# omroot/DeepLearningInAssetPricing_PaperReplication

Measured on AMD Instinct MI355X. Metric: epochs/sec (3-phase GAN), higher is better.
Workload: dtype bf16; 1 GPU; model=Chen-Pelger-Zhu GAN: LSTM[4] + SDF FFN[64,64] + 8 tanh moments, global_batch=1, seq_len=240, panel=T=240/60/300 N=3000 F=46 M=178, bench_config=real, wide_layer0=False, models_per_gpu=1, parallelism=ensemble-dp1, backend=none

## Files before the change

csrc/engine.cpp:

```cpp
#include <cstdint>
#include <cstdlib>
#include <hip/hip_runtime.h>
#include <pybind11/numpy.h>
#include <pybind11/pybind11.h>
#include <pybind11/stl.h>

#include <execinfo.h>
#include <signal.h>
#include <sys/syscall.h>
#include <unistd.h>

#include <atomic>
#include <cmath>
#include <cstring>
#include <map>
#include <memory>
#include <mutex>
#include <stdexcept>
#include <string>
#include <vector>

#include <chrono>

#include "engine_plan.h"
// ... 1472 lines not shown
      launch_mlp_bwd_mom(as<MlpJob>(dh ? j_mlp_bwd_dh_ : j_mlp_bwd_[phase]), G_, gx_bwd_, md_.nslice_m, 1, md_.md,
                         md_.KS1, md_.WMB, slab_stride(), fpw_, st_);
    else
      launch_sdf_bwd(as<MlpJob>(j_mlp_bwd_[phase]));
    if (md_.md.wide)
      launch_wgrad0(as<WideJob>(j_wide_bwd_[phase]), G_, dd(), md_.md, phase == 2, md_.WMB, nsplit_, st_);
    enqueue_train_tail(tp);
  }
  long split_rows(int s) const { return splits_[s].R; }

  void set_stream(uintptr_t st, bool external) {
    HTRACE("set_stream %p ext=%d tid=%ld", (void*)st, (int)external, (long)syscall(SYS_gettid));
    hipStream_t want = external ? reinterpret_cast<hipStream_t>(st) : own_st_;
    if (want == st_ && external == ext_stream_) return;
    sync();
    st_ = want;
    ext_stream_ = external;
  }
  void join_from(uintptr_t ext) {
    HIP_OK(hipEventRecord(ev_[EV_IN], reinterpret_cast<hipStream_t>(ext)));
    HIP_OK(hipStreamWaitEvent(st_, ev_[EV_IN], 0));
  }
  void join_to(uintptr_t ext) {
    HIP_OK(hipEventRecord(ev_[EV_OUT], st_));
    HIP_OK(hipStreamWaitEvent(reinterpret_cast<hipStream_t>(ext), ev_[EV_OUT], 0));
  }
  void set_params_dev(int g, uintptr_t src) {
    check_g(g);
    HIP_OK(hipMemcpyAsync(models_[g].params.p, reinterpret_cast<const void*>(src), md_.P * sizeof(float),
                          hipMemcpyDeviceToDevice, st_));
    pack(g, false);
    h_valid_ = false;
  }
  void set_drop_step(int g, int step) { launch_set_int(models_[check_g(g)].drop_step.p, step, st_); }
  long copy_ws(int g, int s, const std::string& name, uintptr_t dst) {
    ModelSplitWS& W = ws(g, s);
    const std::map<std::string, DevBuf<float>*> m = {
        {"wn", &W.wn}, {"h", &W.h}, {"P", &W.P}, {"port", &W.port}, {"scal", &W.scal}, {"pp", &W.pp},
        {"w", &W.w}};
    auto it = m.find(name);
    if (it == m.end()) throw std::invalid_argument("copy_ws: unknown buffer " + name);
    const DevBuf<float>& b = *it->second;
    if (b.n) HIP_OK(hipMemcpyAsync(reinterpret_cast<void*>(dst), b.p, b.n * sizeof(float), hipMemcpyDeviceToDevice, st_));
    return (long)b.n;
  }
  void copy_grads(int g, uintptr_t dst) {
    HIP_OK(hipMemcpyAsync(reinterpret_cast<void*>(dst), models_[check_g(g)].grads.p, md_.P * sizeof(float),
                          hipMemcpyDeviceToDevice, st_));
  }
  void set_hidden(int g, int s, uintptr_t h, uintptr_t c) {
    ModelSplitWS& W = ws(check_g(g), s);
    const size_t n = (size_t)md_.nrnn * md_.H;
    if (n == 0) return;
    if (h) HIP_OK(hipMemcpyAsync(W.h0.p, reinterpret_cast<const void*>(h), n * 4, hipMemcpyDeviceToDevice, st_));
    else HIP_OK(hipMemsetAsync(W.h0.p, 0, n * 4, st_));
    if (c) HIP_OK(hipMemcpyAsync(W.c0.p, reinterpret_cast<const void*>(c), n * 4, hipMemcpyDeviceToDevice, st_));
    else HIP_OK(hipMemsetAsync(W.c0.p, 0, n * 4, st_));
  }
  void copy_hidden_grad(int g, uintptr_t dh, uintptr_t dc) {
    ModelSplitWS& W = ws(check_g(g), 0);
    const size_t n = (size_t)md_.nrnn * md_.H;
    if (n == 0) return;
    HIP_OK(hipMemcpyAsync(reinterpret_cast<void*>(dh), W.dh0.p, n * 4, hipMemcpyDeviceToDevice, st_));
    HIP_OK(hipMemcpyAsync(reinterpret_cast<void*>(dc), W.dc0.p, n * 4, hipMemcpyDeviceToDevice, st_));
  }
  void copy_hidden(int g, uintptr_t dst_h, uintptr_t dst_c) {
// ... 186 lines not shown
    int gx = std::max(gx_fwd_[1], gx_fwd_[2]);
    if (k_.eval_gx > 0) gx = std::min(gx, k_.eval_gx);
    return gx;
  }
  int train_fwd_grid(int phase) const { return phase == 2 ? gx_fwd_[0] : gx_fwd13_; }
  int ne_per_model() const { return G_ > 0 && n_eval_jobs_ % G_ == 0 ? n_eval_jobs_ / G_ : 0; }
  int tmax_fwd_all() const { return std::max(splits_[0].T, tmax_eval_); }
  bool fused_eval(const EvalPass& ep) const {
    return (k_.rnn_overlap_eval || ep.solo || ep.sep) && plan_[1].eval_fusable;
  }
  void plan_phases() {
    const bool overlap = k_.rnn_overlap && !safe_mode_ && md_.nrnn > 0 && !md_.md.wide;
    auto fits = [&](int T) { return mlp_fwd_rnn_supported(md_.md, md_.KS1, md_.WMB, md_.H, md_.nrnn, T); };
    const bool have0 = splits_[0].set, packs = inv_code_.p != nullptr;
    const int eval_gx = fused_grid(eval_grid(), n_eval_jobs_, cap_eval_), ne = ne_per_model();
    const bool eval_fusable = overlap && n_eval_jobs_ > 0 && fits(tmax_eval_) && eval_gx > 0;
    for (int phase = 1; phase <= 3; ++phase) {
      PhasePlan p;
      p.eval_gx_solo = eval_gx;
      p.eval_fusable = eval_fusable;
      const int gx = fused_grid(train_fwd_grid(phase), G_, cap_train_);
      p.fused_fwd = (phase != 2 || k_.fused_p2) && overlap && fits(splits_[0].T) && gx > 0;
      p.train_gx = p.fused_fwd ? gx : 0;
      p.selfproj = p.fused_fwd && k_.self_proj && !train_mom(phase);
      const int gxa = cap_all_ > 0 && ne > 0 ? std::min(train_fwd_grid(phase), cap_all_ / G_ - 1 - ne) : 0;
      p.eval_in_fwd = k_.eval_in_fwd && phase != 2 && ne > 0 && p.fused_fwd && fits(tmax_fwd_all()) && gxa >= 16;
      p.all_gx = p.eval_in_fwd ? gxa : 0;
      p.sep_eval = k_.eval_sep && phase != 2 && p.fused_fwd && eval_fusable;
      p.tail_fused = k_.fused_tail && !xs_on_ && phase != 2 && have0 && lstm_tail_supported(md_, splits_[0].T);
      const int nadam = (md_.P_sdf + ADAM_PB - 1) / ADAM_PB;
      p.adam_in_tail = k_.tail_adam != 0 && !safe_mode_ && p.tail_fused && packs && tail_cap_ > 0 &&
                       2 * G_ * nadam <= tail_cap_;
      p.split_graphs = k_.split_graphs && !safe_mode_ && p.adam_in_tail && (p.sep_eval || p.eval_in_fwd);
      p.mom_tail = phase == 2 && k_.mom_tail && !xs_on_ && packs && have0 && mom_tail_supported(md_, splits_[0].T) &&
                   !mlstm();
      p.p2_lstm_cached = phase == 2 && k_.p2_lstm_cache && md_.nrnn > 0 && (md_.nrnn == 1 || md_.dropout == 0.f) &&
                         !xs_on_;
      plan_[phase] = p;
    }
  }
  RunMode run_mode(int phase) const {
    const PhasePlan& p = plan_[phase];
    RunMode m;
    m.pipe = phase != 2 && n_eval_jobs_ > 0 && pipeline_;
    m.split = m.pipe && p.split_graphs;
    m.sep = m.split && p.sep_eval;
    m.tail_adam = m.split || (m.pipe && p.eval_in_fwd && k_.tail_adam == 2 && p.adam_in_tail);
    return m;
  }
 public:
  double capture_seconds() const { return capture_s_; }
  bool fused_fwd(int phase) const { return phase >= 1 && phase <= 3 && plan_[phase].fused_fwd; }
  void reset_prog_errors() {
    sync();
    std::vector<int> h((size_t)G_ * 3 * 16);
    HIP_LEGACY(hipMemcpy(h.data(), prog_.p, h.size() * sizeof(int), hipMemcpyDeviceToHost));
    for (int k = 0; k < 3 * G_; ++k) h[16 * k + 1] = 0;
    HIP_LEGACY(hipMemcpy(prog_.p, h.data(), h.size() * sizeof(int), hipMemcpyHostToDevice));
    for (ModelState& S : models_) {
      HIP_LEGACY(hipMemset(S.tail_ctr.p, 0, S.tail_ctr.n * sizeof(int)));
      HIP_LEGACY(hipMemset(S.upd_ctr.p, 0, S.upd_ctr.n * sizeof(int)));
    }
    HIP_LEGACY(hipMemset(esync_.p, 0, esync_.n * sizeof(int)));
  }
  py::dict fused_info() const {
    py::dict d;
    const RunMode m = run_mode(1);
    d["cap_train"] = cap_train_; d["cap_eval"] = cap_eval_;
    for (int ph = 1; ph <= 3; ++ph) d[("train_gx_p" + std::to_string(ph)).c_str()] = plan_[ph].train_gx;
    d["eval_gx_solo"] = plan_[1].eval_gx_solo;
    d["cap_all"] = cap_all_;
    d["tail_cap"] = tail_cap_;
    for (int ph = 1; ph <= 3; ph += 2) {
      d[("eval_in_fwd_p" + std::to_string(ph)).c_str()] = plan_[ph].eval_in_fwd;
      d[("all_gx_p" + std::to_string(ph)).c_str()] = plan_[ph].all_gx;
    }
    d["eval_per_model"] = ne_per_model();
    d["fused_tail"] = plan_[1].tail_fused;
    d["mom_tail"] = plan_[2].mom_tail;
    d["p2_lstm_cached"] = plan_[2].p2_lstm_cached;
    d["adam_in_tail"] = m.tail_adam && plan_[1].eval_in_fwd;
    d["split_graphs"] = m.split;
    d["eval_sep"] = m.sep;
    d["host_launch_us_per_epoch"] = host_launch_n_ ? 1e6 * host_launch_s_ / host_launch_n_ : 0.0;
    d["bwd_nfine"] = nfine_; d["bwd_fpw"] = fpw_;
    d["fused_pack"] = inv_code_.p != nullptr;
    d["bwd_lds_fpw1"] = (long)mlp_bwd_lds_bytes(md_.md, slab_stride(), 1);
    d["bwd_lds_fpw4"] = (long)mlp_bwd_lds_bytes(md_.md, slab_stride(), 4);
    return d;
  }
  int prog_timeouts() {
    sync();
    std::vector<int> h((size_t)G_ * 3 * 16);
    HIP_LEGACY(hipMemcpy(h.data(), prog_.p, h.size() * sizeof(int), hipMemcpyDeviceToHost));
    int n = 0;
    for (int k = 0; k < 3 * G_; ++k) n += h[16 * k + 1];
    return n;
  }
 private:
  bool train_mom(int phase) const { return phase == 2 || (phase == 3 && !cache_train_h()); }
  ModelDesc md_{};
  DevBuf<char> d_desc_;
  SplitDev splits_[3];
  std::vector<ModelState> models_;
  std::vector<ModelSplitWS> ws_;
  DevBuf<float> slab_;
  DevBuf<int> cnt_scratch_;
  DevBuf<float> nbar_scratch_;
  int nfine_ = 4;
  int fpw_ = 1;
  int slabs_stored() const { return nfine_ / fpw_; }
  int gx_bwd_ = 1, gx_fwd_[3] = {1, 1, 1};
  int gx_fwd13_ = 1;
  int nsplit_ = 1, gx_proj_[3] = {1, 1, 1};
  bool graphs_dirty_ = true;
  std::map<std::string, hipGraphExec_t> graphs_;
// ... 803 lines not shown
      HIP_OK(hipEventRecord(ev_[EV_MID], st_));
    } else {
      HTRACE("launch_job_metrics");
      launch_job_metrics(lj, G_, st_);
    }
    if (phase == 2) {
      HTRACE("launch_mlp_bwd_mom");
      launch_mlp_bwd_mom(as<MlpJob>(j_mlp_bwd_[phase]), G_, gx_bwd_, md_.nslice_m, 1, md_.md, md_.KS1,
                         md_.WMB, slab_stride(), fpw_, st_);
    } else {
      if (!tp.gram) {
        HTRACE("launch_period_bwd");
        launch_period_bwd(lj, G_, D.T, st_);
      }
      HTRACE("launch_mlp_bwd_sdf");
      launch_sdf_bwd(as<MlpJob>(j_mlp_bwd_[phase]));
    }
    if (md_.md.wide)
      launch_wgrad0(as<WideJob>(j_wide_bwd_[phase]), G_, dd(), md_.md, phase == 2, md_.WMB, nsplit_, st_);
    enqueue_train_tail(tp);
  }
  void enqueue_train_tail(const TrainPass& tp) {
    const int phase = tp.phase;
    const SplitDev& D = splits_[0];
    if (tp.mom_adam) {
      HTRACE("launch_lstm_tail(phase 2)");
      launch_lstm_tail(as<UpdJob>(j_upd_), as<FinJob>(j_fin_), G_, dd(), md_, D.T, slab_stride(), st_,
                       loss_tab(2, false), 1, tp.lr, 2);
      return;
    }
    const LossJob* lm = tp.tail_metrics && phase != 2 ? loss_tab(phase, tp.gram) : nullptr;
    if (plan_[phase].tail_fused) {
      HTRACE("launch_lstm_tail");
      launch_lstm_tail(as<UpdJob>(j_upd_), as<FinJob>(j_fin_), G_, dd(), md_, D.T, slab_stride(), st_, lm,
                       tp.tail_adam, tp.lr);
      return;
    }
    if (lm) launch_job_metrics(lm, G_, st_);
    HTRACE("launch_finalize");
    launch_finalize(as<FinJob>(j_fin_), G_, dd(), md_, phase, slab_stride(), D.T, st_);
    xs_call("grads", phase, st_);
    if (phase == 2 && mlstm()) {
      HTRACE("launch_mlstm_bwd");
      launch_mlstm_bwd(as<MlstmJob>(j_ml_train_), G_, D.T, dd(), md_, st_);
      return;
    }
    HTRACE("launch_lstm_bwd");
    launch_lstm_bwd(as<UpdJob>(j_upd_), G_, dd(), md_, D.T, phase, st_);
  }
  void enqueue_update(int phase, float lr) {
    HTRACE("launch_update");
    launch_update(as<UpdJob>(j_upd_), G_, dd(), md_, phase, lr, st_, inv_code_.p != nullptr);
  }
  void enqueue_train(int phase, float lr) {
    enqueue_train_grads(TrainPass(phase));
    enqueue_update(phase, lr);
  }
  void enqueue_eval(hipStream_t st, const EvalPass& ep) {
    enqueue_eval_prologue(st, ep);
    enqueue_eval_towers(st, ep);
  }
  void enqueue_eval_prologue(hipStream_t st, const EvalPass& ep) {
    if (n_eval_jobs_ == 0) return;
    HTRACE("launch_prologue");
    if (fused_eval(ep)) launch_proj(as<RnnJob>(j_rnn_eval_), n_eval_jobs_, tmax_eval_, dd(), md_, st, proj_abias(!k_.h_cache));
    else launch_prologue(as<RnnJob>(j_rnn_eval_), n_eval_jobs_, tmax_eval_, dd(), md_, st, proj_abias(!k_.h_cache));
    mom_table(j_ml_eval_, 0, n_eval_jobs_, tmax_eval_, st, !k_.h_cache, false);
  }
// ... 29 lines not shown
  void enqueue_eval_solo(int phase) {
    EvalPass ep = eval_pass(phase);
    ep.solo = true;
    enqueue_eval(st_, ep);
  }
  void enqueue_epoch_end(int phase, int ignore_epoch, float sel, hipStream_t st, int signal = 0) {
    HTRACE("launch_epoch_end");
    launch_epoch_end(as<EpochJob>(j_epoch_[phase]), G_, phase, ignore_epoch, sel, md_.residual_factor,
                     md_.P, st, signal);
  }
  void enqueue_epoch(int phase, float lr, int ignore_epoch, float sel, bool lstm_once) {
    TrainPass tp = epoch_pass(phase, lr);
    tp.mom_adam = plan_[phase].mom_tail;
    tp.lstm_once = lstm_once;
    enqueue_train_grads(tp);
    if (!tp.mom_adam) enqueue_update(phase, lr);
    if (phase != 2) enqueue_eval_solo(phase);
    enqueue_epoch_end(phase, ignore_epoch, sel, st_);
  }
  void enqueue_head(int phase, float lr, int part) {
    TrainPass tp = epoch_pass(phase, lr);
    tp.part = part;
    enqueue_train_grads(tp);
    enqueue_dropmask(phase, 1, st_);
    enqueue_update(phase, lr);
    if (plan_[phase].split_graphs && plan_[phase].sep_eval) launch_gen_sync(as<UpdJob>(j_upd_), G_, st_);
  }
  void enqueue_chain_split(int phase, float lr) {
    const bool sep = plan_[phase].sep_eval;
    TrainPass tp = epoch_pass(phase, lr);
    tp.premasked = true;
    tp.tail_metrics = true;
    tp.tail_adam = sep ? 3 : 2;
    tp.eval_rnn = !sep;
    tp.esig = sep ? nullptr : esync_.p;
    enqueue_train_grads(tp);
  }
  void enqueue_eval_split(int phase, int ignore_epoch, float sel) {
    EvalPass ep = eval_pass(phase);
    if (plan_[phase].sep_eval) {
      HTRACE("launch_wait_gen");
      launch_wait_gen(as<UpdJob>(j_upd_), G_, k_.spin_limit, st2_);
      ep.sep = true;
      ep.selfproj = k_.self_proj && k_.h_cache;
      if (!ep.selfproj) launch_proj(as<RnnJob>(j_rnn_eval_), n_eval_jobs_, tmax_eval_, dd(), md_, st2_, proj_abias(!k_.h_cache));
      mom_table(j_ml_eval_, 0, n_eval_jobs_, tmax_eval_, st2_, !k_.h_cache, false);
    } else {
      HTRACE("launch_wait_count");
      launch_wait_count(esync_.p, ne_per_model() * G_, k_.spin_limit, prog_.p, G_, st2_);
    }
    enqueue_eval_towers(st2_, ep);
    enqueue_dropmask(phase, 1, st2_);
    enqueue_epoch_end(phase, ignore_epoch, sel, st2_, 1);
  }
  void enqueue_pipe(int phase, float lr, int ignore_epoch, float sel) {
    HIP_OK(hipEventRecord(ev_[EV_FORK], st_));
    HIP_OK(hipStreamWaitEvent(st2_, ev_[EV_FORK], 0));
    TrainPass tp = epoch_pass(phase, lr);
    tp.premasked = true;
    const EvalPass ep = eval_pass(phase);
    if (plan_[phase].eval_in_fwd) {
      const bool ta = run_mode(phase).tail_adam;
      tp.eval_rnn = tp.mark_fwd = tp.tail_metrics = true;
      tp.tail_adam = ta ? 2 : 0;
      enqueue_train_grads(tp);
      HIP_OK(hipStreamWaitEvent(st2_, ev_[EV_FWD], 0));
      enqueue_eval_towers(st2_, ep);
      if (ta) {
        enqueue_dropmask(phase, 1, st2_);
        enqueue_epoch_end(phase, ignore_epoch, sel, st2_, 1);
        HIP_OK(hipEventRecord(ev_[EV_JOIN], st2_));
        HIP_OK(hipStreamWaitEvent(st_, ev_[EV_JOIN], 0));
        return;
      }
      enqueue_epoch_end(phase, ignore_epoch, sel, st2_);
      enqueue_dropmask(phase, 1, st2_);
    } else {
      tp.eval_prologue = st2_;
      tp.defer_metrics = true;
      enqueue_train_grads(tp);
      enqueue_eval_towers(st2_, ep);
      if (phase != 2) {
        HIP_OK(hipStreamWaitEvent(st2_, ev_[EV_MID], 0));
        launch_job_metrics(loss_tab(phase, tp.gram), G_, st2_);
      }
// ... 295 lines not shown
      .def("characteristic_gram", &Engine::characteristic_gram, py::arg("s"))
      .def("xgram_run", &Engine::xgram_run)
      .def("pred_loss", &Engine::pred_loss, py::arg("s"), py::arg("factor") = py::none(),
           py::arg("weighting") = "period", py::arg("refresh") = true, py::arg("write_dw") = false)
      .def("fit_begin", &Engine::fit_begin, py::arg("factors"), py::arg("weighting") = "period")
      .def("fit_epochs", &Engine::fit_epochs, py::arg("n"), py::arg("lr"), py::call_guard<py::gil_scoped_release>())
      .def("fit_history", &Engine::fit_history)
      .def("fit_best", &Engine::fit_best)
      .def("fit_load_best", &Engine::fit_load_best)
      .def("apply_update", &Engine::apply_update)
      .def("weight_surface", &Engine::weight_surface, py::arg("s"), py::arg("scale"), py::arg("grid"), py::arg("base"),
           py::arg("items"), py::arg("refresh") = true)
      .def("weight_surface_supported", [](Engine& e, int s) { return e.wsurf_ok(s); }, py::arg("s") = 0)
      .def("knockout", &Engine::knockout, py::arg("s"), py::arg("masks"), py::arg("n_scen"), py::arg("base"),
           py::arg("w_out") = 0, py::arg("refresh") = true, py::arg("max_scratch_bytes") = 0, py::arg("raw_out") = 0,
           py::arg("raw_in") = 0)
      .def("knockout_supported", [](Engine& e, int s) { return e.knock_ok(s); }, py::arg("s") = 0)
      .def("knockout_macro", &Engine::knockout_macro, py::arg("s"), py::arg("masks"), py::arg("macro_masks"),
           py::arg("n_scen"), py::arg("base"), py::arg("macro_base"), py::arg("w_out") = 0, py::arg("refresh") = true,
           py::arg("max_scratch_bytes") = 0, py::arg("raw_out") = 0)
      .def("knockout_macro_supported", [](Engine& e, int s) { return e.knock_macro_ok(s); }, py::arg("s") = 0)
      .def("train_step", &Engine::train_step)
      .def("backward_only", &Engine::backward_only, py::arg("phase"), py::arg("wait") = true)
      .def("set_stream", &Engine::set_stream, py::arg("stream"), py::arg("external") = true)
      .def("set_params_dev", &Engine::set_params_dev)
      .def("join_from", &Engine::join_from)
      .def("xs_backward", &Engine::xs_backward, py::arg("phase"), py::arg("dw"), py::arg("dE"), py::arg("sdf"),
           py::arg("dh") = 0)
      .def("set_hidden", &Engine::set_hidden)
      .def("copy_hidden_grad", &Engine::copy_hidden_grad)
      .def("split_rows", &Engine::split_rows)
      .def("join_to", &Engine::join_to)
      .def("set_drop_step", &Engine::set_drop_step)
      .def("copy_ws", &Engine::copy_ws)
      .def("copy_grads", &Engine::copy_grads)
      .def("copy_hidden", &Engine::copy_hidden)
      .def("read_ws", &Engine::read_ws)
      .def("read_aux", &Engine::read_aux)
      .def("read_gram", &Engine::read_gram)
      .def("refresh_gram", &Engine::refresh_gram)
      .def("gram_enabled", &Engine::gram_enabled)
      .def("read_blob", &Engine::read_blob)
      .def("sync", &Engine::sync, py::call_guard<py::gil_scoped_release>())
      .def("stream", &Engine::stream);
  m.def("ensemble_portfolios",
        [](uintptr_t W, int G, int T, int N, uintptr_t R, uintptr_t mask, uintptr_t port, uintptr_t port_ind,
           uintptr_t stream) {
          launch_ensemble(reinterpret_cast<const float*>(W), G, T, N, reinterpret_cast<const float*>(R),
                          reinterpret_cast<const float*>(mask), reinterpret_cast<float*>(port),
                          reinterpret_cast<float*>(port_ind), reinterpret_cast<hipStream_t>(stream));
        },
        "K11: ensemble portfolio [T] and individual portfolios [G][T] from gathered weights (device pointers)");
  m.def("rank_characteristics",
        [](uintptr_t x, uintptr_t rowok, uintptr_t out, uintptr_t cnt, long long T, int N, int F, float thr,
           float fill_missing, float fill_dead, uintptr_t stream) {
          launch_xrank(reinterpret_cast<const float*>(x), reinterpret_cast<const uint8_t*>(rowok),
                       reinterpret_cast<float*>(out), reinterpret_cast<int*>(cnt), T, N, F, thr, fill_missing,
                       fill_dead, reinterpret_cast<hipStream_t>(stream));
        },
        py::arg("x"), py::arg("rowok"), py::arg("out"), py::arg("cnt"), py::arg("T"), py::arg("N"), py::arg("F"),
        py::arg("thr"), py::arg("fill_missing"), py::arg("fill_dead"), py::arg("stream") = 0,
        "cross-sectional rank transform of a dense fp32 chunk [T][N][F] (device pointers; out may be x)");
  m.def("rank_supported", [](int N) { return xrank_supported(N); });
  m.def("rank_block_keys", []() { return xrank_block_keys(); });
  m.attr("XRANK_MAX_N") = (int)XRANK_MAX_N;
  m.def("characteristic_moments",
// ... 25 lines not shown
```

csrc/engine_plan.h:

```cpp
#pragma once
#include <hip/hip_runtime.h>

#include <algorithm>
#include <cstdlib>

inline int grid_per_model(int one, int lo, int G) { return std::max(lo, one / std::max(1, G)); }

inline int env_int(const char* name, int dflt) {
  const char* v = std::getenv(name);
  return v && *v ? std::atoi(v) : dflt;
}

struct Knobs {
  bool rnn_overlap;
  bool rnn_overlap_eval;
  bool fused_p2;
  bool eval_in_fwd;
  bool eval_sep;
  bool self_proj;
  bool fused_tail;
  bool mom_tail;
  int tail_adam;
  bool split_graphs;
  int unroll;
  bool p2_lstm_cache;
  bool train_gram_side;
  bool h_cache;
  bool gram;
  int gram_plan;
  bool fused_pack;
  int prog_mode;
  unsigned spin_limit;
  int fused_cap;
  bool wide;
  int tps;
  bool tbwd;
  int eval_gx;
  bool zx_eval, zx_train;
  int zx_gx;
  int gx_fwd;
  int gx_fwd13;
  int gx_proj;
  int wg_split;
  int nslab_coarse;
  int bwd_fpw;
  bool pp_global;
};

inline Knobs read_knobs(int G, bool fp32) {
  Knobs k{};
  k.rnn_overlap = env_int("DLAP_RNN_OVERLAP", 1) != 0;
  k.rnn_overlap_eval = env_int("DLAP_RNN_OVERLAP_EVAL", 0) != 0;
  k.fused_p2 = env_int("DLAP_FUSED_PHASE2", 0) != 0;
  k.eval_in_fwd = env_int("DLAP_EVAL_IN_FWD", 1) != 0;
  k.eval_sep = env_int("DLAP_EVAL_SEP", 0) != 0;
  k.self_proj = env_int("DLAP_SELF_PROJ", 1) != 0;
  k.fused_tail = env_int("DLAP_FUSED_TAIL", 1) != 0;
  k.mom_tail = env_int("DLAP_MOM_TAIL", 1) != 0;
  k.tail_adam = env_int("DLAP_TAIL_ADAM", 1);
  k.split_graphs = env_int("DLAP_SPLIT_GRAPHS", 1) != 0;
  k.unroll = std::max(1, env_int("DLAP_UNROLL", 8));
  k.p2_lstm_cache = env_int("DLAP_P2_LSTM_CACHE", 1) != 0;
  k.train_gram_side = env_int("DLAP_TRAIN_GRAM_SIDE", 0) != 0;
  k.h_cache = env_int("DLAP_H_CACHE", 1) != 0;
  k.gram = env_int("DLAP_GRAM", 1) != 0;
  k.gram_plan = env_int("DLAP_GRAM_PLAN", 1);
  k.fused_pack = env_int("DLAP_FUSED_PACK", 1) != 0;
  k.prog_mode = env_int("DLAP_PROG_MODE", 1);
  k.spin_limit = (unsigned)env_int("DLAP_PROG_SPIN_LIMIT", 1 << 22);
  k.fused_cap = env_int("DLAP_FUSED_CAP", -1);
  k.wide = env_int("DLAP_WIDE", 0) != 0;
  k.tps = env_int("DLAP_TPS", 1);
  k.tbwd = env_int("DLAP_TBWD", 1) != 0;
  k.eval_gx = env_int("DLAP_EVAL_GX", grid_per_model(256, 64, G));
  k.zx_eval = !fp32 && env_int("DLAP_ZX_EVAL", 1) != 0;
  k.zx_train = !fp32 && env_int("DLAP_ZX_TRAIN", 1) != 0;
  k.zx_gx = std::max(1, env_int("DLAP_ZX_GX", 256));
  k.gx_fwd = env_int("DLAP_GX_FWD", G <= 2 ? 1024 : grid_per_model(1024, 128, G));
  k.gx_fwd13 = env_int("DLAP_GX_FWD13", grid_per_model(384, 96, G));
  k.gx_proj = env_int("DLAP_GX_PROJ", 512);
  k.wg_split = env_int("DLAP_WG_SPLIT", 512);
  k.nslab_coarse = env_int("DLAP_NSLAB_COARSE", 64);
  k.bwd_fpw = env_int("DLAP_BWD_FPW", 1);
  k.pp_global = env_int("DLAP_PP_GLOBAL", 0) != 0;
  return k;
}

struct PhasePlan {
  bool fused_fwd = false;
  int train_gx = 0;
  bool eval_in_fwd = false;
  int all_gx = 0;
  bool selfproj = false;
  bool sep_eval = false;
  bool tail_fused = false;
  bool adam_in_tail = false;
  bool split_graphs = false;
  bool mom_tail = false;
  bool p2_lstm_cached = false;
  bool eval_fusable = false;
  int eval_gx_solo = 0;
};

struct RunMode {
  bool pipe = false;
  bool split = false;
  bool sep = false;
  bool tail_adam = false;
};

struct TrainPass {
  explicit TrainPass(int phase_, float lr_ = 0.f) : phase(phase_), lr(lr_) {}
  int phase;
  float lr;
  bool gram = false;
  int part = 0;
  bool premasked = false;
  bool own_proj = true;
  bool eval_rnn = false;
  int* esig = nullptr;
  hipStream_t eval_prologue = nullptr;
  bool lstm_once = false;
  bool mark_fwd = false;
  bool defer_metrics = false;
  bool tail_metrics = false;
  int tail_adam = 0;
  bool mom_adam = false;
};

struct EvalPass {
  bool gram = false;
  bool solo = false;
  bool sep = false;
  bool selfproj = false;
};
```

csrc/k_mlp.hip:

```cpp
#include <algorithm>
#include "common.h"
#include "layout.h"
#include "mlp.h"
#include "lstm_gls.h"
#include "tower_dev.h"

#ifndef DLAP_FWD_WPS
#define DLAP_FWD_WPS 2
#endif

#ifndef DLAP_BWD1_WPS
#define DLAP_BWD1_WPS 2
#endif

__device__ long long g_mlp_ts[24];
#define MLP_TS(slot) do { \
    if ((threadIdx.x & 255) == 0 && (bx == 0 || bx == gxw - 1) && J.gbits) \
      g_mlp_ts[(bx == 0 ? 0 : 4) + (slot)] = wall_clock64(); } while (0)

template <class P, int WMB, typename L0>
DLAP_DEV void mom_forward_tile(const typename P::Frag* lds, const float* aux, const MlpDims& D,
                               const MlpJob& J, const DropCtx& dc, const RowInfo& ri, L0&& layer0_fn) {
  constexpr int KSM = (WMB + 1) / 2;
  f32x4 a[2][WMB];
  typename P::Frag pf[2][KSM];
  const int q = lane_id() >> 4;
  layer0_fn(a);
  for (int j = 0; j + 1 < D.nl_mom; ++j) {
    const uint32_t kw = dc.on ? hash_keep<WMB>(dc, 16 + j, ri) : 0xFFFFFFFFu;
    act_tile_rt<P, WMB>(a, dc.on, kw, pf);
    layer_chain<P, WMB, KSM>(lds, D.m_fwd + j * WMB * KSM, pf, a, aux + D.a_mb + 64 * (j + 1));
  }
#pragma unroll
  for (int b = 0; b < 2; ++b) {
    if (ri.dense[b] < 0) continue;
    const auto dst = gp(J.h_out) + (size_t)ri.dense[b] * D.K;
#pragma unroll
    for (int u = 0; u < WMB; ++u)
// ... 886 lines not shown
  }
  float* red = wg_slab_begin(sred, slab_stride);
  for (int w = 0; w < nwaves; ++w) {
    if (wave == w) {
#pragma unroll
      for (int t = 0; t < TPS; ++t)
#pragma unroll
        for (int u = 0; u < WMB; ++u)
#pragma unroll
          for (int v = 0; v < 4; ++v)
#pragma unroll
            for (int r = 0; r < 4; ++r)
              red[t * 4096 + (16 * u + 4 * q + r) * 64 + ((16 * v + (lane & 15)) ^ ((q & 1) << 4))] += dW[t][u][v][r];
      if (slice == 0) {
        float* ex = red + TPS * 4096;
        const int jl = lane & 15;
#pragma unroll
        for (int u = 0; u < WMB; ++u)
#pragma unroll
          for (int r = 0; r < 4; ++r)
            if (jl < DLAP_MAXL) ex[jl * 64 + ((16 * u + 4 * q + r + 5 * jl) & 63)] += gbias[u][r];
      }
    }
    __syncthreads();
  }
  wg_slab_finish<TPS, 0>(J, red, slab_stride, kf);
  }
}

__global__ __launch_bounds__(256) void k_dropmask(const MlpJob* __restrict__ jobs, MlpDims D, int step_offset) {
  const MlpJob& J = jobs[blockIdx.y];
  const int ntiles = (J.R + 31) >> 5;
  const int gid = blockIdx.x * 256 + threadIdx.x;
  const int tile = gid >> 6, lane = gid & 63, q = lane >> 4;
  if (tile >= ntiles) return;
  const uint32_t step = (J.step ? (uint32_t)*gp(J.step) : 0u) + (uint32_t)step_offset;
  if (!(J.dropout > 0.f)) return;
  const uint32_t thr16 = (uint32_t)(J.dropout * 65536.f + 0.5f);
  uint32_t rowmix[2];
#pragma unroll
  for (int b = 0; b < 2; ++b) {
    const int r = tile * 32 + 16 * b + (lane & 15);
    const int2 ti = gp(J.rowti)[min(r, J.R - 1)];
    rowmix[b] = row_mix(r < J.R ? (uint32_t)(ti.x * J.N + ti.y) : 0xFFFFFFFFu);
  }
  const auto dst = gp(const_cast<uint32_t*>(J.gbits)) + (size_t)(step & 1u) * J.gb_half + (size_t)tile * D.nl_sdf * 64 + lane;
  for (int j = 0; j < D.nl_sdf; ++j) dst[64 * j] = keep_word<4>(dropout_key(J.seed, step, j), rowmix, thr16, q);
}

void launch_dropmask(const MlpJob* jobs, int njobs, int ntiles, const MlpDims& D, int step_offset,
                     hipStream_t st) {
  hipLaunchKernelGGL(k_dropmask, dim3((ntiles * 64 + 255) / 256, njobs), dim3(256), 0, st, jobs, D,
                     step_offset);
  HIP_OK(hipGetLastError());
}

size_t mlp_lds_bytes(const MlpDims& D) { return lds_bytes_of(D); }
static size_t bwd_red_off(const MlpDims& D, int ) {
  return (mlp_lds_bytes(D) + 15) & ~(size_t)15;
}
bool mlp_bwd_fpw_fits(const MlpDims& D, int KS1, int slab_stride, int tps, int fpw) {
  if (fpw > 1 && !D.wide && !(KS1 == 2 && tps == 1)) return false;
  const size_t per_cu = 160 * 1024 / (tps == 1 ? DLAP_BWD1_WPS : 1);
  return mlp_bwd_lds_bytes(D, slab_stride, fpw) <= per_cu;
}
size_t mlp_bwd_lds_bytes(const MlpDims& D, int slab_stride, int fpw) {
  const size_t a = mlp_lds_bytes(D), b = (size_t)slab_stride * 4;
  return fpw > 1 ? bwd_red_off(D, slab_stride) + 2 * b : (a > b ? a : b);
}

template <class P>
static bool launch_mlp_fwd_p(const MlpJob* jobs, dim3 grid, dim3 block, size_t sh, const MlpDims& D, int KS1,
                             int WMB, hipStream_t st, bool so) {
  if (so && !P::kF32) {
    if (KS1 == 2) { hipLaunchKernelGGL((k_mlp_fwd<P, 2, 1, false, true>), grid, block, sh, st, jobs, D); HIP_OK(hipGetLastError()); return true; }
    if (KS1 == 4) { hipLaunchKernelGGL((k_mlp_fwd<P, 4, 1, false, true>), grid, block, sh, st, jobs, D); HIP_OK(hipGetLastError()); return true; }
  }
#define F_CASE(K, W) if (KS1 == K && WMB == W) { hipLaunchKernelGGL((k_mlp_fwd<P, K, W, false>), grid, block, sh, st, jobs, D); HIP_OK(hipGetLastError()); return true; }
  F_CASE(2, 1) F_CASE(2, 2) F_CASE(2, 4) F_CASE(4, 1) F_CASE(4, 2) F_CASE(4, 4)
#undef F_CASE
// ... 173 lines not shown
```

csrc/k_rnn.hip:

```cpp
#include <algorithm>
#include <cstdlib>
#include "common.h"
#include "layout.h"
#include "rnn.h"
#include "update.h"
#include "lstm_gls.h"
#include "finalize.h"
#include "loss_dev.h"
#include "pack_dev.h"

#define DLAP_MAX_M 1024

__device__ long long g_rnn_ts[24];
#define RNN_TS(slot, cond) do { if ((cond) && threadIdx.x == 0) g_rnn_ts[slot] = wall_clock64(); } while (0)

DLAP_DEV float sigm(float x) { return __builtin_amdgcn_rcpf(1.f + __expf(-x)); }
DLAP_DEV float ftanh(float x) {
  const float t = 2.f * sigm(2.f * x) - 1.f;
  return fabsf(x) < 0.0125f ? x * (1.f - x * x * (1.f / 3.f)) : t;
}

__global__ __launch_bounds__(64) void k_proj(const RnnJob* __restrict__ jobs,
                                             const ModelDesc* __restrict__ md, int y0) {
  const RnnJob& J = jobs[blockIdx.z];
  const int T = J.T;
  const int t0 = blockIdx.x * 16, o0 = (blockIdx.y + y0) * 16;
  const int G4 = md->nrnn > 0 ? 4 * md->H : 0;
  if (t0 >= T) return;
  if (o0 >= G4 && !J.abias) return;
  const bool tsm = blockIdx.x == 0 && blockIdx.y == 0 && blockIdx.z == 0;
  RNN_TS(12, tsm);
  if (J.prog && blockIdx.x == 0 && blockIdx.y == 0 && threadIdx.x == 0) gp(J.prog)[0] = 0;
  const f32x4 acc = proj_tile(J, md, t0, o0);
  const int l = threadIdx.x, n = l & 15, kq = l >> 4;
  const int o = o0 + n;
#pragma unroll
  for (int r = 0; r < 4; ++r) {
    const int t = t0 + 4 * kq + r;
    if (t >= T) break;
    const float v = acc[r];
    if (o < G4) gp(J.xg)[(size_t)t * G4 + o] = v;
    else if (o - G4 < 64) gp(J.abias)[t * 64 + (o - G4)] = v;
// ... 984 lines not shown
      while (ok && evgen && (unsigned)__builtin_amdgcn_readfirstlane(__hip_atomic_load(gen, __ATOMIC_RELAXED, __HIP_MEMORY_SCOPE_AGENT)) -
                           (k + 1) > 0x7fffffffu) {
        if (spins++ >= U.spin_limit) { ok = false; break; }
        __builtin_amdgcn_s_sleep(2);
      }
      asm volatile("" ::: "memory");
      __builtin_amdgcn_fence(__ATOMIC_ACQUIRE, "agent");
      asm volatile("s_waitcnt vmcnt(0)" ::: "memory");
      if (threadIdx.x == 0) {
        if (!ok) atomicAdd(const_cast<int*>(U.prog) + 1, 1);
        s_go = ok && !prog_poisoned(U.prog);
      }
    }
    __syncthreads();
    RNN_TS(19, tsm && bx == 0);
    return s_go != 0;
  };
  adam_block(U, md, phase, lr, bx, nadam, red, wait, step_pre, drop_pre);
  if (gen) {
    __syncthreads();
    if (threadIdx.x == 0) {
      const unsigned prev = __hip_atomic_fetch_add(reinterpret_cast<unsigned*>(U.tail_ctr + TAIL_ADONE), 1u,
                                                   __ATOMIC_ACQ_REL, __HIP_MEMORY_SCOPE_AGENT);
      if ((prev + 1u) % (unsigned)nadam == 0u)
        __hip_atomic_fetch_add(U.tail_ctr + TAIL_UPDGEN, 1, __ATOMIC_RELEASE, __HIP_MEMORY_SCOPE_AGENT);
    }
  }
  RNN_TS(20, tsm && bx == nadam - 1);
}

template <int HM, int WPS>
__global__ __launch_bounds__(256, WPS) void k_lstm_tail(const UpdJob* __restrict__ ujobs, const FinJob* __restrict__ fjobs,
                                                   const ModelDesc* __restrict__ md, int slab_stride, int nslab_blocks,
                                                   const LossJob* __restrict__ ljobs, int adam, float lr, int phase) {
  extern __shared__ __attribute__((aligned(16))) float sm[];
  const UpdJob& U = ujobs[blockIdx.y];
  const FinJob& F = fjobs[blockIdx.y];
  const int b = (int)blockIdx.x - 1;
  const int nwg = (md->M + 1 + 15) / 16;
  const bool mom = phase == 2;
  __shared__ int s_steps[2];
  if (adam && threadIdx.x == 0) { s_steps[0] = gp(U.adam_step)[mom ? 1 : 0]; s_steps[1] = gp(U.drop_step)[0]; }
  if (b < 0 && mom) {
    __shared__ int bad;
    if (threadIdx.x < 64) {
      const int* ctr = U.tail_ctr + TAIL_CNT;
      unsigned spins = 0;
      bool ok = true;
      while (__builtin_amdgcn_readfirstlane(__hip_atomic_load(ctr, __ATOMIC_RELAXED, __HIP_MEMORY_SCOPE_AGENT)) < U.T) {
        if (spins++ >= U.spin_limit) { ok = false; break; }
        __builtin_amdgcn_s_sleep(2);
      }
      asm volatile("" ::: "memory");
      __builtin_amdgcn_fence(__ATOMIC_ACQUIRE, "agent");
      if (threadIdx.x == 0) {
        bad = ok ? 0 : 1;
        if (!ok) atomicAdd(const_cast<int*>(U.prog) + 1, 1);
        else {
          __hip_atomic_store(U.tail_ctr + TAIL_CNT, 0, __ATOMIC_RELAXED, __HIP_MEMORY_SCOPE_AGENT);
          __builtin_amdgcn_fence(__ATOMIC_RELEASE, "agent");
          __hip_atomic_store(U.tail_ctr + TAIL_FLAG, 1, __ATOMIC_RELAXED, __HIP_MEMORY_SCOPE_AGENT);
        }
      }
    }
    __syncthreads();
  } else if (b < 0) {
    lstm_bwd_body<HM, true>(U, md, 1, sm, blockIdx.y == 0);
  } else if (b < U.T) {
    finalize_block(F, md, phase, slab_stride, nslab_blocks + b, U.tail_ctr + TAIL_CNT);
  } else if (b < U.T + nslab_blocks) {
    finalize_block(F, md, phase, slab_stride, b - U.T);
  } else if (b >= U.T + nslab_blocks + nwg) {
    if (ljobs) job_metrics_body<256>(ljobs[blockIdx.y], sm + DLAP_MAX_T, sm);
  } else {
    const int cblk = b - U.T - nslab_blocks;
    __shared__ int bad;
    auto wait_dg = [&]() -> bool {
      if (threadIdx.x < 64) {
        const int* flag = U.tail_ctr + TAIL_FLAG;
        int v = __builtin_amdgcn_readfirstlane(__hip_atomic_load(flag, __ATOMIC_RELAXED, __HIP_MEMORY_SCOPE_AGENT));
        unsigned spins = 0;
        bool ok = true;
        while (v == 0) {
          if (spins++ >= U.spin_limit) { ok = false; break; }
          __builtin_amdgcn_s_sleep(2);
          v = __builtin_amdgcn_readfirstlane(__hip_atomic_load(flag, __ATOMIC_RELAXED, __HIP_MEMORY_SCOPE_AGENT));
        }
        asm volatile("" ::: "memory");
        __builtin_amdgcn_fence(__ATOMIC_ACQUIRE, "agent");
        asm volatile("s_waitcnt vmcnt(0)" ::: "memory");
        if (threadIdx.x == 0) bad = ok ? 0 : 1;
      }
      __syncthreads();
      return bad == 0;
    };
    f32x4* red = reinterpret_cast<f32x4*>(sm);
    const int G = mom ? md->m[0].out : 4 * md->H;
    if (G <= 16) wgrad_block<1>(U, md, phase, cblk, red, U.tail_ctr + TAIL_DONE, nwg, wait_dg);
    else if (G <= 32) wgrad_block<2>(U, md, phase, cblk, red, U.tail_ctr + TAIL_DONE, nwg, wait_dg);
    else wgrad_block<4>(U, md, phase, cblk, red, U.tail_ctr + TAIL_DONE, nwg, wait_dg);
    if (blockIdx.y == 0 && cblk == nwg - 1 && threadIdx.x == 0) g_rnn_ts[17] = wall_clock64();
  }
  if (adam) tail_adam(U, md, lr, gridDim.x, s_steps[0], s_steps[1], phase, adam >= 2, adam == 3);
}

static bool tail_dense(const ModelDesc& mh) { return mh.H == 4; }
size_t lstm_tail_lds_bytes(const ModelDesc& mh, int T) {
  return lstm_bwd_lds(T, mh.H, false, tail_dense(mh)).total * sizeof(float);
}
bool lstm_tail_supported(const ModelDesc& mh, int T) {
  if (mh.nrnn < 1 || mh.H > 8 || mh.M <= 0 || T < 2) return false;
  const char* scan_env = std::getenv("DLAP_LSTM_SCAN");
  if (tail_dense(mh) && scan_env && std::atoi(scan_env) == 0) return false;
  const size_t lim = tail_dense(mh) ? 80 * 1024 : 160 * 1024;
  return lstm_tail_lds_bytes(mh, T) + 6400 <= lim;
}
int lstm_tail_words() { return TAIL_WORDS; }
static size_t tail_dyn_lds(const ModelDesc& mh, int T, int phase = 1) {
  const size_t small = std::max((size_t)(DLAP_MAX_T + 4) * sizeof(float), (size_t)4 * 4 * 64 * 16);
  return phase == 2 ? small : std::max(lstm_tail_lds_bytes(mh, T), small);
}
bool mom_tail_supported(const ModelDesc& mh, int T) {
  return mh.M > 0 && mh.m[0].out <= 64 && T >= 1;
}
static bool tail_one_wave(const ModelDesc& mh, int njobs) { return mh.H <= 4 && njobs == 1; }
int lstm_tail_capacity(const ModelDesc& mh, int T, int njobs) {
  const size_t sh = tail_dyn_lds(mh, T);
  int per_cu = 0, dev = 0, ncu = 0;
  if (tail_one_wave(mh, njobs)) HIP_OK(hipOccupancyMaxActiveBlocksPerMultiprocessor(&per_cu, k_lstm_tail<4, 1>, 256, sh));
  else if (mh.H <= 4) HIP_OK(hipOccupancyMaxActiveBlocksPerMultiprocessor(&per_cu, k_lstm_tail<4, 2>, 256, sh));
  else HIP_OK(hipOccupancyMaxActiveBlocksPerMultiprocessor(&per_cu, k_lstm_tail<8, 2>, 256, sh));
  HIP_OK(hipGetDevice(&dev));
  HIP_OK(hipDeviceGetAttribute(&ncu, hipDeviceAttributeMultiprocessorCount, dev));
  return per_cu * ncu;
}
void launch_lstm_tail(const UpdJob* ujobs, const FinJob* fjobs, int njobs, const ModelDesc* md, const ModelDesc& mh,
                      int T, int slab_stride, hipStream_t st, const LossJob* ljobs, int adam, float lr, int phase) {
  const int nslab_blocks = (phase == 2 ? mh.ntile_m : mh.ntile_s) * 64 + (SLAB_EXTRA + 63) / 64;
  const int nwg = (mh.M + 1 + 15) / 16;
  const size_t sh = tail_dyn_lds(mh, T, phase);
  const dim3 grid(1 + T + nslab_blocks + nwg + (ljobs ? 1 : 0), njobs);
  if (tail_one_wave(mh, njobs))
    hipLaunchKernelGGL((k_lstm_tail<4, 1>), grid, dim3(256), sh, st, ujobs, fjobs, md, slab_stride, nslab_blocks, ljobs, adam,
                       lr, phase);
  else if (mh.H <= 4)
    hipLaunchKernelGGL((k_lstm_tail<4, 2>), grid, dim3(256), sh, st, ujobs, fjobs, md, slab_stride, nslab_blocks, ljobs, adam,
                       lr, phase);
  else
    hipLaunchKernelGGL((k_lstm_tail<8, 2>), grid, dim3(256), sh, st, ujobs, fjobs, md, slab_stride, nslab_blocks, ljobs, adam,
                       lr, phase);
  HIP_OK(hipGetLastError());
}

void launch_lstm_bwd(const UpdJob* jobs, int njobs, const ModelDesc* md, const ModelDesc& mh,
                     int T, int phase, hipStream_t st) {
  if (phase != 2 && mh.nrnn > 0) {
    size_t sh = ((size_t)T * (LSTM_NCOEF + 2 + 4) * mh.H + 64 + lstm_gpart_floats(mh.H)) * sizeof(float);
    if (sh > 160 * 1024) dlap_throw_hip(hipErrorInvalidValue, "lstm_bwd: T*H too large for LDS", __FILE__, __LINE__);
    const char* scan_env = std::getenv("DLAP_LSTM_SCAN");
    const bool scan_on = !(scan_env && std::atoi(scan_env) == 0);
    const size_t sh_scan = sh + lstm_bwd_scan_floats(T) * sizeof(float);
    const int scan = scan_on && mh.H == 4 && T >= 2 && sh_scan <= 160 * 1024 ? 1 : 0;
    if (scan) sh = sh_scan;
    if (mh.H <= 4) hipLaunchKernelGGL((k_lstm_bwd<4>), dim3(njobs), dim3(256), sh, st, jobs, md, scan);
    else if (mh.H <= 8) hipLaunchKernelGGL((k_lstm_bwd<8>), dim3(njobs), dim3(256), sh, st, jobs, md, 0);
    else if (mh.H <= 16) hipLaunchKernelGGL((k_lstm_bwd<16>), dim3(njobs), dim3(256), sh, st, jobs, md, 0);
    else hipLaunchKernelGGL((k_lstm_bwd<32>), dim3(njobs), dim3(256), sh, st, jobs, md, 0);
    HIP_OK(hipGetLastError());
  }
  if (mh.M == 0) return;
  if (phase != 2 && mh.nrnn == 0) return;
  const int G = phase == 2 ? mh.m[0].out : 4 * mh.H;
  dim3 grid((mh.M + 1 + 15) / 16, njobs);
  if (G <= 16) hipLaunchKernelGGL((k_wgrad<1>), grid, dim3(256), 0, st, jobs, md, phase);
  else if (G <= 32) hipLaunchKernelGGL((k_wgrad<2>), grid, dim3(256), 0, st, jobs, md, phase);
  else if (G <= 64) hipLaunchKernelGGL((k_wgrad<4>), grid, dim3(256), 0, st, jobs, md, phase);
  else hipLaunchKernelGGL((k_wgrad<8>), grid, dim3(256), 0, st, jobs, md, phase);
  HIP_OK(hipGetLastError());
}

std::vector<long long> rnn_timestamps() {
  std::vector<long long> v(24);
  HIP_OK(hipMemcpyFromSymbol(v.data(), HIP_SYMBOL(g_rnn_ts), sizeof(long long) * 24));
// ... 3 lines not shown
```

csrc/update.h:

```cpp
#pragma once
#include "common.h"

struct ModelDesc;

#define PACK_FAN 4
#define ADAM_PB 1024
#define TAIL_CNT 0
#define TAIL_FLAG 32
#define TAIL_DONE 64
#define TAIL_ARRIVE 96
#define TAIL_EVGEN 128
#define TAIL_ARRIVE2 160
#define TAIL_ADONE 192
#define TAIL_UPDGEN 224
#define TAIL_UPDSEEN 256
#define TAIL_WORDS 288

struct FinJob {
  const float* slab;
  float* grads;
  const int* row_ptr;
  const float* u;
  float* dpp;
  const float* v;
// ... 46 lines not shown
  H_PHASE = 0, H_TRAIN_LOSS, H_TRAIN_SHARPE, H_VALID_LOSS, H_VALID_SHARPE, H_TEST_LOSS,
  H_TEST_SHARPE, H_TRAIN_LUNC, H_TRAIN_LCOND, H_GNORM, H_VALID_LUNC, H_VALID_LCOND,
  H_VALID_MDD, H_VALID_MEAN, H_VALID_STD, H_TEST_LUNC, H_TEST_LCOND, H_TEST_MDD,
  H_TEST_MEAN, H_TEST_STD, H_TRAIN_LRES, H_BEST_LOSS, H_BEST_SR, H_SNAP, HIST_W = 24
};

struct EpochJob {
  const float* sc_train;
  const float* sc_valid;
  const float* sc_test;
  const float* gnorm;
  float* hist;
  int* ep;
  float* best;
  int* snap_flags;
  const float* params;
  float* snap_loss;
  float* snap_sharpe;
  int max_ep;
  const int* prog;
  int* eval_gen;
};

void launch_finalize(const FinJob* jobs, int njobs, const ModelDesc* md, const ModelDesc& mh,
                     int phase, int slab_stride, int tmax, hipStream_t st, int part = 0);
void launch_update(const UpdJob* jobs, int njobs, const ModelDesc* md, const ModelDesc& mh, int phase,
                   float lr, hipStream_t st, bool fused);
void launch_lstm_bwd(const UpdJob* jobs, int njobs, const ModelDesc* md, const ModelDesc& mh,
                     int T, int phase, hipStream_t st);
bool lstm_tail_supported(const ModelDesc& mh, int T);
int lstm_tail_words();
int lstm_tail_capacity(const ModelDesc& mh, int T, int njobs);
struct LossJob;
void launch_lstm_tail(const UpdJob* ujobs, const FinJob* fjobs, int njobs, const ModelDesc* md, const ModelDesc& mh,
                      int T, int slab_stride, hipStream_t st, const LossJob* ljobs = nullptr, int adam = 0,
                      float lr = 0.f, int phase = 1);
bool mom_tail_supported(const ModelDesc& mh, int T);
void launch_pack(float* const* params_unused, const UpdJob* jobs, int njobs, const ModelDesc* md,
                 const ModelDesc& mh, hipStream_t st);
int pack_total(const ModelDesc& mh);
void pack_index_host(const ModelDesc& mh, int* src);
void launch_set_int(int* p, int v, hipStream_t st);
void launch_begin_phase(const EpochJob* jobs, int njobs, hipStream_t st);
void launch_wait_count(int* cnt, int per, unsigned limit, int* prog, int nmodels, hipStream_t st);
void launch_wait_gen(const UpdJob* jobs, int njobs, unsigned limit, hipStream_t st);
void launch_gen_sync(const UpdJob* jobs, int njobs, hipStream_t st);
void launch_epoch_end(const EpochJob* jobs, int njobs, int phase, int ignore_epoch, float sel,
                      float res_factor, int P, hipStream_t st, int signal = 0);
```

Baseline: 7439 model-epochs/s.

## Generate next-step dropout masks inside the fused LSTM tail kernel

Result: faster. 7537 model-epochs/s, median of 6 (+1.3%).

```diff
diff --git a/csrc/dropmask_dev.h b/csrc/dropmask_dev.h
--- /dev/null
+++ b/csrc/dropmask_dev.h
@@ -0,0 +1,29 @@
+#pragma once
+#include "mlp.h"
+
+template <int U>
+DLAP_DEV void dropmask_tiles(const MlpJob& J, int nl_sdf, uint32_t step, int tile0, int stride, int tile_end,
+                             int lane) {
+  const int q = lane >> 4;
+  const uint32_t thr16 = (uint32_t)(J.dropout * 65536.f + 0.5f);
+  int2 ti[U][2];
+#pragma unroll
+  for (int u = 0; u < U; ++u) {
+    const int tile = min(tile0 + u * stride, tile_end - 1);
+#pragma unroll
+    for (int b = 0; b < 2; ++b) ti[u][b] = gp(J.rowti)[min(tile * 32 + 16 * b + (lane & 15), J.R - 1)];
+  }
+#pragma unroll
+  for (int u = 0; u < U; ++u) {
+    const int tile = tile0 + u * stride;
+    if (tile >= tile_end) break;
+    uint32_t rowmix[2];
+#pragma unroll
+    for (int b = 0; b < 2; ++b) {
+      const int r = tile * 32 + 16 * b + (lane & 15);
+      rowmix[b] = row_mix(r < J.R ? (uint32_t)(ti[u][b].x * J.N + ti[u][b].y) : 0xFFFFFFFFu);
+    }
+    const auto dst = gp(const_cast<uint32_t*>(J.gbits)) + (size_t)(step & 1u) * J.gb_half + (size_t)tile * nl_sdf * 64 + lane;
+    for (int j = 0; j < nl_sdf; ++j) dst[64 * j] = keep_word<4>(dropout_key(J.seed, step, j), rowmix, thr16, q);
+  }
+}
diff --git a/csrc/engine.cpp b/csrc/engine.cpp
--- a/csrc/engine.cpp
+++ b/csrc/engine.cpp
@@ -1528,6 +1528,18 @@
     pack(g, false);
     h_valid_ = false;
   }
+  py::array_t<uint32_t> keep_words(int g, int parity) {
+    ensure_jobs();
+    check_g(g);
+    if (parity < 0 || parity > 1) throw std::invalid_argument("parity must be 0 or 1");
+    const size_t half = (size_t)((splits_[0].R + 31) / 32) * md_.nl_s * 64;
+    sync();
+    py::array_t<uint32_t> out((py::ssize_t)half);
+    if (ws(g, 0).gb.n < 2 * half) throw std::runtime_error("keep_words: no keep words allocated for this split");
+    if (half)
+      HIP_LEGACY(hipMemcpy(out.mutable_data(), ws(g, 0).gb.p + (size_t)parity * half, half * sizeof(uint32_t), hipMemcpyDeviceToHost));
+    return out;
+  }
   void set_drop_step(int g, int step) { launch_set_int(models_[check_g(g)].drop_step.p, step, st_); }
   long copy_ws(int g, int s, const std::string& name, uintptr_t dst) {
     ModelSplitWS& W = ws(g, s);
@@ -1780,6 +1792,12 @@
       p.adam_in_tail = k_.tail_adam != 0 && !safe_mode_ && p.tail_fused && packs && tail_cap_ > 0 &&
                        2 * G_ * nadam <= tail_cap_;
       p.split_graphs = k_.split_graphs && !safe_mode_ && p.adam_in_tail && (p.sep_eval || p.eval_in_fwd);
+      p.tail_masks = k_.tail_masks != 0 && p.split_graphs && md_.dropout > 0.f && md_.H == 4 && md_.nrnn == 1 &&
+                     (G_ == 1 || k_.tail_masks > 1);
+      if (p.tail_masks) {
+        const int ntiles = (splits_[0].R + 31) / 32;
+        p.mask_blocks = k_.tail_masks > 1 ? std::min(k_.tail_masks, ntiles) : std::max(1, std::min((ntiles + 15) / 16, 224));
+      }
       p.mom_tail = phase == 2 && k_.mom_tail && !xs_on_ && packs && have0 && mom_tail_supported(md_, splits_[0].T) &&
                    !mlstm();
       p.p2_lstm_cached = phase == 2 && k_.p2_lstm_cache && md_.nrnn > 0 && (md_.nrnn == 1 || md_.dropout == 0.f) &&
@@ -1830,6 +1848,8 @@
     d["adam_in_tail"] = m.tail_adam && plan_[1].eval_in_fwd;
     d["split_graphs"] = m.split;
     d["eval_sep"] = m.sep;
+    d["tail_masks"] = m.split && plan_[1].tail_masks;
+    d["tail_mask_blocks"] = m.split && plan_[1].tail_masks ? plan_[1].mask_blocks : 0;
     d["host_launch_us_per_epoch"] = host_launch_n_ ? 1e6 * host_launch_s_ / host_launch_n_ : 0.0;
     d["bwd_nfine"] = nfine_; d["bwd_fpw"] = fpw_;
     d["fused_pack"] = inv_code_.p != nullptr;
@@ -2699,8 +2719,10 @@
     const LossJob* lm = tp.tail_metrics && phase != 2 ? loss_tab(phase, tp.gram) : nullptr;
     if (plan_[phase].tail_fused) {
       HTRACE("launch_lstm_tail");
+      const bool masks = tp.tail_masks && tp.tail_adam != 0;
       launch_lstm_tail(as<UpdJob>(j_upd_), as<FinJob>(j_fin_), G_, dd(), md_, D.T, slab_stride(), st_, lm,
-                       tp.tail_adam, tp.lr);
+                       tp.tail_adam, tp.lr, 1, masks ? as<MlpJob>(j_mlp_train_[phase]) : nullptr, md_.md.nl_sdf,
+                       masks ? plan_[phase].mask_blocks : 0);
       return;
     }
     if (lm) launch_job_metrics(lm, G_, st_);
@@ -2796,6 +2818,7 @@
     tp.premasked = true;
     tp.tail_metrics = true;
     tp.tail_adam = sep ? 3 : 2;
+    tp.tail_masks = plan_[phase].tail_masks;
     tp.eval_rnn = !sep;
     tp.esig = sep ? nullptr : esync_.p;
     enqueue_train_grads(tp);
@@ -2814,7 +2837,7 @@
       launch_wait_count(esync_.p, ne_per_model() * G_, k_.spin_limit, prog_.p, G_, st2_);
     }
     enqueue_eval_towers(st2_, ep);
-    enqueue_dropmask(phase, 1, st2_);
+    if (!plan_[phase].tail_masks) enqueue_dropmask(phase, 1, st2_);
     enqueue_epoch_end(phase, ignore_epoch, sel, st2_, 1);
   }
   void enqueue_pipe(int phase, float lr, int ignore_epoch, float sel) {
@@ -3176,6 +3199,7 @@
       .def("split_rows", &Engine::split_rows)
       .def("join_to", &Engine::join_to)
       .def("set_drop_step", &Engine::set_drop_step)
+      .def("keep_words", &Engine::keep_words)
       .def("copy_ws", &Engine::copy_ws)
       .def("copy_grads", &Engine::copy_grads)
       .def("copy_hidden", &Engine::copy_hidden)
diff --git a/csrc/engine_plan.h b/csrc/engine_plan.h
--- a/csrc/engine_plan.h
+++ b/csrc/engine_plan.h
@@ -29,6 +29,7 @@
   bool gram;
   int gram_plan;
   bool fused_pack;
+  int tail_masks;
   int prog_mode;
   unsigned spin_limit;
   int fused_cap;
@@ -66,6 +67,7 @@
   k.gram = env_int("DLAP_GRAM", 1) != 0;
   k.gram_plan = env_int("DLAP_GRAM_PLAN", 1);
   k.fused_pack = env_int("DLAP_FUSED_PACK", 1) != 0;
+  k.tail_masks = std::max(0, env_int("DLAP_TAIL_MASKS", 1));
   k.prog_mode = env_int("DLAP_PROG_MODE", 1);
   k.spin_limit = (unsigned)env_int("DLAP_PROG_SPIN_LIMIT", 1 << 22);
   k.fused_cap = env_int("DLAP_FUSED_CAP", -1);
@@ -96,6 +98,8 @@
   bool tail_fused = false;
   bool adam_in_tail = false;
   bool split_graphs = false;
+  bool tail_masks = false;
+  int mask_blocks = 0;
   bool mom_tail = false;
   bool p2_lstm_cached = false;
   bool eval_fusable = false;
@@ -125,6 +129,7 @@
   bool defer_metrics = false;
   bool tail_metrics = false;
   int tail_adam = 0;
+  bool tail_masks = false;
   bool mom_adam = false;
 };
 
diff --git a/csrc/k_mlp.hip b/csrc/k_mlp.hip
--- a/csrc/k_mlp.hip
+++ b/csrc/k_mlp.hip
@@ -4,6 +4,7 @@
 #include "mlp.h"
 #include "lstm_gls.h"
 #include "tower_dev.h"
+#include "dropmask_dev.h"
 
 #ifndef DLAP_FWD_WPS
 #define DLAP_FWD_WPS 2
@@ -956,20 +957,11 @@
   const MlpJob& J = jobs[blockIdx.y];
   const int ntiles = (J.R + 31) >> 5;
   const int gid = blockIdx.x * 256 + threadIdx.x;
-  const int tile = gid >> 6, lane = gid & 63, q = lane >> 4;
+  const int tile = gid >> 6, lane = gid & 63;
   if (tile >= ntiles) return;
   const uint32_t step = (J.step ? (uint32_t)*gp(J.step) : 0u) + (uint32_t)step_offset;
   if (!(J.dropout > 0.f)) return;
-  const uint32_t thr16 = (uint32_t)(J.dropout * 65536.f + 0.5f);
-  uint32_t rowmix[2];
-#pragma unroll
-  for (int b = 0; b < 2; ++b) {
-    const int r = tile * 32 + 16 * b + (lane & 15);
-    const int2 ti = gp(J.rowti)[min(r, J.R - 1)];
-    rowmix[b] = row_mix(r < J.R ? (uint32_t)(ti.x * J.N + ti.y) : 0xFFFFFFFFu);
-  }
-  const auto dst = gp(const_cast<uint32_t*>(J.gbits)) + (size_t)(step & 1u) * J.gb_half + (size_t)tile * D.nl_sdf * 64 + lane;
-  for (int j = 0; j < D.nl_sdf; ++j) dst[64 * j] = keep_word<4>(dropout_key(J.seed, step, j), rowmix, thr16, q);
+  dropmask_tiles<1>(J, D.nl_sdf, step, tile, 1, ntiles, lane);
 }
 
 void launch_dropmask(const MlpJob* jobs, int njobs, int ntiles, const MlpDims& D, int step_offset,
diff --git a/csrc/k_rnn.hip b/csrc/k_rnn.hip
--- a/csrc/k_rnn.hip
+++ b/csrc/k_rnn.hip
@@ -8,6 +8,7 @@
 #include "finalize.h"
 #include "loss_dev.h"
 #include "pack_dev.h"
+#include "dropmask_dev.h"
 
 #define DLAP_MAX_M 1024
 
@@ -1058,7 +1059,8 @@
 template <int HM, int WPS>
 __global__ __launch_bounds__(256, WPS) void k_lstm_tail(const UpdJob* __restrict__ ujobs, const FinJob* __restrict__ fjobs,
                                                    const ModelDesc* __restrict__ md, int slab_stride, int nslab_blocks,
-                                                   const LossJob* __restrict__ ljobs, int adam, float lr, int phase) {
+                                                   const LossJob* __restrict__ ljobs, int adam, float lr, int phase,
+                                                   const MlpJob* __restrict__ mjobs, int nl_sdf, int nmask) {
   extern __shared__ __attribute__((aligned(16))) float sm[];
   const UpdJob& U = ujobs[blockIdx.y];
   const FinJob& F = fjobs[blockIdx.y];
@@ -1097,7 +1099,23 @@
   } else if (b < U.T + nslab_blocks) {
     finalize_block(F, md, phase, slab_stride, b - U.T);
   } else if (b >= U.T + nslab_blocks + nwg) {
-    if (ljobs) job_metrics_body<256>(ljobs[blockIdx.y], sm + DLAP_MAX_T, sm);
+    const int mb = b - (U.T + nslab_blocks + nwg) - (ljobs ? 1 : 0);
+    if (mb < 0) {
+      job_metrics_body<256>(ljobs[blockIdx.y], sm + DLAP_MAX_T, sm);
+    } else if (mjobs) {
+      const MlpJob& MJ = mjobs[blockIdx.y];
+      __syncthreads();
+      RNN_TS(21, blockIdx.y == 0 && mb == 0);
+      if (MJ.dropout > 0.f) {
+        const int ntiles = (MJ.R + 31) >> 5, per = (ntiles + nmask - 1) / nmask;
+        const int lo = mb * per, hi = min(lo + per, ntiles);
+        const uint32_t step = (uint32_t)s_steps[1] + 1u;
+        constexpr int MU = 4;
+        for (int t0 = lo + (int)(threadIdx.x >> 6); t0 < hi; t0 += 4 * MU)
+          dropmask_tiles<MU>(MJ, nl_sdf, step, t0, 4, hi, threadIdx.x & 63);
+      }
+      RNN_TS(22, blockIdx.y == 0 && mb == nmask - 1);
+    }
   } else {
     const int cblk = b - U.T - nslab_blocks;
     __shared__ int bad;
@@ -1161,20 +1179,23 @@
   return per_cu * ncu;
 }
 void launch_lstm_tail(const UpdJob* ujobs, const FinJob* fjobs, int njobs, const ModelDesc* md, const ModelDesc& mh,
-                      int T, int slab_stride, hipStream_t st, const LossJob* ljobs, int adam, float lr, int phase) {
+                      int T, int slab_stride, hipStream_t st, const LossJob* ljobs, int adam, float lr, int phase,
+                      const MlpJob* mjobs, int nl_sdf, int nmask) {
+  if (!mjobs || !adam || phase == 2 || nmask < 0) nmask = 0;
+  if (nmask == 0) mjobs = nullptr;
   const int nslab_blocks = (phase == 2 ? mh.ntile_m : mh.ntile_s) * 64 + (SLAB_EXTRA + 63) / 64;
   const int nwg = (mh.M + 1 + 15) / 16;
   const size_t sh = tail_dyn_lds(mh, T, phase);
-  const dim3 grid(1 + T + nslab_blocks + nwg + (ljobs ? 1 : 0), njobs);
+  const dim3 grid(1 + T + nslab_blocks + nwg + (ljobs ? 1 : 0) + nmask, njobs);
   if (tail_one_wave(mh, njobs))
     hipLaunchKernelGGL((k_lstm_tail<4, 1>), grid, dim3(256), sh, st, ujobs, fjobs, md, slab_stride, nslab_blocks, ljobs, adam,
-                       lr, phase);
+                       lr, phase, mjobs, nl_sdf, nmask);
   else if (mh.H <= 4)
     hipLaunchKernelGGL((k_lstm_tail<4, 2>), grid, dim3(256), sh, st, ujobs, fjobs, md, slab_stride, nslab_blocks, ljobs, adam,
-                       lr, phase);
+                       lr, phase, mjobs, nl_sdf, nmask);
   else
     hipLaunchKernelGGL((k_lstm_tail<8, 2>), grid, dim3(256), sh, st, ujobs, fjobs, md, slab_stride, nslab_blocks, ljobs, adam,
-                       lr, phase);
+                       lr, phase, mjobs, nl_sdf, nmask);
   HIP_OK(hipGetLastError());
 }
 
diff --git a/csrc/update.h b/csrc/update.h
--- a/csrc/update.h
+++ b/csrc/update.h
@@ -102,9 +102,10 @@
 int lstm_tail_words();
 int lstm_tail_capacity(const ModelDesc& mh, int T, int njobs);
 struct LossJob;
+struct MlpJob;
 void launch_lstm_tail(const UpdJob* ujobs, const FinJob* fjobs, int njobs, const ModelDesc* md, const ModelDesc& mh,
                       int T, int slab_stride, hipStream_t st, const LossJob* ljobs = nullptr, int adam = 0,
-                      float lr = 0.f, int phase = 1);
+                      float lr = 0.f, int phase = 1, const MlpJob* mjobs = nullptr, int nl_sdf = 0, int nmask = 0);
 bool mom_tail_supported(const ModelDesc& mh, int T);
 void launch_pack(float* const* params_unused, const UpdJob* jobs, int njobs, const ModelDesc* md,
                  const ModelDesc& mh, hipStream_t st);
```
